# 18281818221/kalle-audio

Hardware: AMD Instinct MI355X
Metric: audio-seconds/sec (node) DiT train step, 10s@12.5Hz x1024 latents (higher is better)
Workload: dtype bf16; 1 GPU; DiT train step (fwd+bwd+allreduce+Adam), 24 blocks D=1536 h=24, 10 s @ 12.5 Hz x 1024 latents (T=125+1 prepend), S=130 x 768 cross-attn cond; DiT shape chosen by this build (reference defines none); global_batch=256, per_gpu_batch=256, parallelism=dp1, objective=v, io_channels=1024, global_cond_type=prepend

## Files before the change

kalle_audio_amd/csrc/gemm2.hip:

```cpp
#include <stdio.h>
#include <stdlib.h>
#include <string.h>

#include <algorithm>
#include <functional>
#include <type_traits>
#include <utility>

#include "gemm_common.h"
#include "../../include/kalle_hip.h"

namespace {

constexpr int BK2 = 64;
#define GPTR(p) ((const __attribute__((address_space(1))) void*)(p))

__device__ __attribute__((aligned(64))) const unsigned kalle_zero_block[16] = {0, 0, 0, 0, 0, 0, 0, 0, 0, 0, 0, 0, 0, 0, 0, 0};

template <bool KM, int R, int NW>
struct Loader {
    static constexpr int PER_WAVE = (R / 8) / NW;
    const bf16_t* src[PER_WAVE];
    int64_t kstep;

// ... 51 lines not shown
            __builtin_amdgcn_global_load_lds(GPTR(sp), LDS_PTR(void, region + (wave * PER_WAVE + i) * 1024), 16, 0, 0);
            src[i] += kstep;
        }
    }
    __device__ __forceinline__ void issue_at(char* region, int wave, int lane, int t, int tail_t, int kvalid) {
        if (t == tail_t) issue_tail(region, wave, lane, kvalid);
        else issue(region, wave);
    }
};

template <int OFF>
__device__ __forceinline__ i32x4 lds_b128(unsigned a) {
    i32x4 r;
    asm volatile("ds_read_b128 %0, %1 offset:%2" : "=v"(r) : "v"(a), "n"(OFF));
    return r;
}
__device__ __forceinline__ i32x2 lds_tr(unsigned a) {
    i32x2 r;
    asm volatile("ds_read_b64_tr_b16 %0, %1" : "=v"(r) : "v"(a));
    return r;
}

template <bool KM, int R>
struct Reader {
    unsigned b0[2], b1[2];
    __device__ __forceinline__ void init(int region_off, int rbase, int lane) {
#pragma unroll
        for (int s = 0; s < 2; ++s) {
            if constexpr (!KM) {
                const int row = rbase + (lane & 15);
                const int c = 4 * s + (lane >> 4);
                b0[s] = region_off + row * 128 + ((c ^ ((row >> 1) & 7)) << 4);
                b1[s] = 0;
            } else {
                constexpr int RB = 2 * R;
                const int g = lane >> 4, i = lane & 15;
                const int q = i >> 2, pp = i & 3;
                const int b = 4 * s + g;
                const int odd = b & 1;
                const int pos1 = 8 * b + (odd ? 4 : 0) + q;
                const int pos2 = 8 * b + (odd ? 0 : 4) + q;
                const int cl = (rbase >> 3) + (pp >> 1);
                const int hb = (pp & 1) * 8;
                b0[s] = region_off + pos1 * RB + ((cl ^ (2 * (pos1 & 7))) << 4) + hb;
                b1[s] = region_off + pos2 * RB + ((cl ^ (2 * (pos2 & 7))) << 4) + hb;
            }
        }
    }
    template <int S, int NTILE, int T0 = 0>
    __device__ __forceinline__ void read(unsigned so, i32x4 (&f)[NTILE]) const {
        if constexpr (!KM) {
            const unsigned a = b0[S] + so;
            f[0] = lds_b128<2048 * (T0 + 0)>(a);
            f[1] = lds_b128<2048 * (T0 + 1)>(a);
            f[2] = lds_b128<2048 * (T0 + 2)>(a);
            f[3] = lds_b128<2048 * (T0 + 3)>(a);
            if constexpr (NTILE == 8) {
                f[4] = lds_b128<2048 * (T0 + 4)>(a);
                f[5] = lds_b128<2048 * (T0 + 5)>(a);
                f[6] = lds_b128<2048 * (T0 + 6)>(a);
                f[7] = lds_b128<2048 * (T0 + 7)>(a);
            }
        } else {
            const unsigned a0 = b0[S] + so, a1 = b1[S] + so;
#pragma unroll
            for (int t = 0; t < NTILE; ++t) {
                const i32x2 lo = lds_tr(a0 ^ ((T0 + t) << 5));
                const i32x2 hi = lds_tr(a1 ^ ((T0 + t) << 5));
                f[t] = i32x4{lo[0], lo[1], hi[0], hi[1]};
            }
        }
    }
};

__device__ __forceinline__ void gemm_stamp(const GemmParams& p, int wave, int lane, int idx, int slot = -1) {
    if (p.stamps && (wave == 0 || wave == 7) && lane == 0)
        p.stamps[((int64_t)(slot < 0 ? (int)blockIdx.x : slot) * 2 + (wave ? 1 : 0)) * 8 + idx] = __builtin_amdgcn_s_memrealtime();
}

constexpr int EPI_DEPTH = 1;

struct NoHook { __device__ __forceinline__ void operator()() const {} };

__device__ __forceinline__ int pidx(int r, int c) { return r * 64 + (c ^ ((r & 1) << 2)); }

template <bool C_F32, int TM, int GLU = 0, typename Hook = NoHook>
__device__ __forceinline__ void wave_epilogue(const GemmParams& p, f32x4 (&acc)[TM][4], char* patch_base, int wave, int lane,
                                              int row0, int col0, Hook after_barrier = Hook{}, int stamp_slot = -1) {
    constexpr int DEPTH = EPI_DEPTH < TM ? EPI_DEPTH : TM;
    float* patch = reinterpret_cast<float*>(patch_base) + wave * (16 * 64);
    const int g = lane >> 4, li = lane & 15;
    const bool pre_res = C_F32 && GLU == 0 && !p.atomic && p.residual != nullptr;
    f32x4 rbuf[DEPTH][4];
    auto load_res = [&](int mt, f32x4 (&rv)[4]) {
#pragma unroll
        for (int i = 0; i < 4; ++i) {
            const int gm = row0 + 16 * mt + g + 4 * i, gn = col0 + 4 * li;
            rv[i] = f32x4{0.f, 0.f, 0.f, 0.f};
            if (gm < p.M && gn < p.N) rv[i] = *reinterpret_cast<const f32x4*>(p.residual + gemm_crow(p, gm) * p.ldr + gn);
        }
    };
    i32x4 hbuf[DEPTH][2][2];
    auto load_h = [&](int mt, i32x4 (&hv)[2][2]) {
        const int c8 = (lane & 7) * 8, j0 = col0 + c8;
#pragma unroll
        for (int half = 0; half < 2; ++half) {
            const int gm = row0 + 16 * mt + (lane >> 3) + 8 * half;
            hv[half][0] = i32x4{0, 0, 0, 0};
            hv[half][1] = i32x4{0, 0, 0, 0};
            if (gm < p.M && j0 < p.glu_inner) {
                const bf16_t* hp = static_cast<const bf16_t*>(p.glu_aux) + (int64_t)gm * 2 * p.glu_inner;
                hv[half][0] = *reinterpret_cast<const i32x4*>(hp + j0);
                hv[half][1] = *reinterpret_cast<const i32x4*>(hp + p.glu_inner + j0);
            }
        }
    };
    asm volatile("s_waitcnt lgkmcnt(0)" ::: "memory");
    __builtin_amdgcn_s_barrier();
    after_barrier();
    gemm_stamp(p, wave, lane, 3, stamp_slot);
#pragma unroll
    for (int d = 0; d < DEPTH; ++d) {
        if constexpr (GLU == 2) load_h(d, hbuf[d]);
        if (pre_res) load_res(d, rbuf[d]);
    }
    float sx[8], sg[8];
#pragma unroll
    for (int e = 0; e < 8; ++e) { sx[e] = 0.f; sg[e] = 0.f; }
    f32x4 bias4 = f32x4{0.f, 0.f, 0.f, 0.f}, bias8[2] = {f32x4{0.f, 0.f, 0.f, 0.f}, f32x4{0.f, 0.f, 0.f, 0.f}};
    float bx[8], bg[8];
#pragma unroll
    for (int e = 0; e < 8; ++e) { bx[e] = 0.f; bg[e] = 0.f; }
    if (p.bias) {
        if constexpr (GLU == 1) {
            const int j0 = col0 + (lane & 3) * 8;
            if (j0 < p.glu_inner) {
#pragma unroll
                for (int e = 0; e < 8; ++e) { bx[e] = p.bias[j0 + e]; bg[e] = p.bias[p.glu_inner + j0 + e]; }
            }
        } else if constexpr (GLU == 0) {
            if constexpr (C_F32) {
                if (!p.atomic && col0 + 4 * li < p.N) bias4 = *reinterpret_cast<const f32x4*>(p.bias + col0 + 4 * li);
            } else {
                const int gn = col0 + 8 * (lane & 7);
                if (gn < p.N) {
                    bias8[0] = *reinterpret_cast<const f32x4*>(p.bias + gn);
                    bias8[1] = *reinterpret_cast<const f32x4*>(p.bias + gn + 4);
                }
            }
        }
    }
#pragma unroll
    for (int mt = 0; mt < TM; ++mt) {
        const int slot = mt % DEPTH;
        f32x4 rcur[4];
        i32x4 hcur[2][2];
        if constexpr (GLU == 2) {
#pragma unroll
            for (int half = 0; half < 2; ++half) { hcur[half][0] = hbuf[slot][half][0]; hcur[half][1] = hbuf[slot][half][1]; }
            if (mt + DEPTH < TM) load_h(mt + DEPTH, hbuf[slot]);
        }
        if (pre_res) {
#pragma unroll
            for (int i = 0; i < 4; ++i) rcur[i] = rbuf[slot][i];
            if (mt + DEPTH < TM) load_res(mt + DEPTH, rbuf[slot]);
        }
#pragma unroll
        for (int nt = 0; nt < 4; ++nt)
#pragma unroll
            for (int r = 0; r < 4; ++r) patch[pidx(4 * g + r, 16 * nt + li)] = acc[mt][nt][r];
        asm volatile("s_waitcnt lgkmcnt(0)" ::: "memory");
        const int rbase = row0 + 16 * mt;
        if constexpr (GLU == 1) {
            const int r = lane >> 2, c8 = (lane & 3) * 8;
            const int gm = rbase + r, j0 = col0 + c8;
            if (gm < p.M && j0 < p.glu_inner) {
                float xv[8], gv[8];
#pragma unroll
                for (int e = 0; e < 8; ++e) { xv[e] = patch[pidx(r, c8 + e)]; gv[e] = patch[pidx(r, 32 + c8 + e)]; }
#pragma unroll
                for (int e = 0; e < 8; ++e) { xv[e] += bx[e]; gv[e] += bg[e]; }
                i32x4 hx, hg, av;
#pragma unroll
                for (int e = 0; e < 4; ++e) {
                    hx[e] = (int)pack_bf16x2(xv[2 * e], xv[2 * e + 1]);
                    hg[e] = (int)pack_bf16x2(gv[2 * e], gv[2 * e + 1]);
                    const float x0 = bf16lo((uint32_t)hx[e]), x1 = bf16hi((uint32_t)hx[e]);
                    const float g0 = bf16lo((uint32_t)hg[e]), g1 = bf16hi((uint32_t)hg[e]);
                    av[e] = (int)pack_bf16x2(x0 * siluf_(g0), x1 * siluf_(g1));
                }
                bf16_t* hp = reinterpret_cast<bf16_t*>(p.C) + (int64_t)gm * p.ldc;
                *reinterpret_cast<i32x4*>(hp + j0) = hx;
                *reinterpret_cast<i32x4*>(hp + p.glu_inner + j0) = hg;
                *reinterpret_cast<i32x4*>(static_cast<bf16_t*>(p.glu_aux) + (int64_t)gm * p.glu_inner + j0) = av;
            }
        } else if constexpr (GLU == 2) {
            const int c8 = (lane & 7) * 8, j0 = col0 + c8;
#pragma unroll
            for (int half = 0; half < 2; ++half) {
                const int r = (lane >> 3) + 8 * half;
                const int gm = rbase + r;
                if (gm < p.M && j0 < p.glu_inner) {
                    const i32x4 xv = hcur[half][0], gv = hcur[half][1];
                    i32x4 ox, og;
#pragma unroll
                    for (int e = 0; e < 4; ++e) {
                        const float x[2] = {bf16lo((uint32_t)xv[e]), bf16hi((uint32_t)xv[e])};
                        const float gg[2] = {bf16lo((uint32_t)gv[e]), bf16hi((uint32_t)gv[e])};
                        const float d[2] = {bf16_to_f32(f32_to_bf16(patch[pidx(r, c8 + 2 * e)] * p.alpha)),
                                            bf16_to_f32(f32_to_bf16(patch[pidx(r, c8 + 2 * e + 1)] * p.alpha))};
                        float dx[2], dg[2];
#pragma unroll
                        for (int q = 0; q < 2; ++q) {
                            const float sgm = sigmoidf_(gg[q]);
                            dx[q] = d[q] * gg[q] * sgm;
                            dg[q] = d[q] * x[q] * sgm * (1.f + gg[q] * (1.f - sgm));
                        }
                        ox[e] = (int)pack_bf16x2(dx[0], dx[1]);
                        og[e] = (int)pack_bf16x2(dg[0], dg[1]);
                        sx[2 * e] += bf16lo((uint32_t)ox[e]); sx[2 * e + 1] += bf16hi((uint32_t)ox[e]);
                        sg[2 * e] += bf16lo((uint32_t)og[e]); sg[2 * e + 1] += bf16hi((uint32_t)og[e]);
                    }
                    bf16_t* dp = reinterpret_cast<bf16_t*>(p.C) + (int64_t)gm * p.ldc;
                    *reinterpret_cast<i32x4*>(dp + j0) = ox;
                    *reinterpret_cast<i32x4*>(dp + p.glu_inner + j0) = og;
                }
            }
        } else if (p.atomic) {
            const int gn = col0 + lane;
#pragma unroll 4
            for (int r = 0; r < 16; ++r) {
                const int gm = rbase + r;
                if (gm < p.M && gn < p.N)
                    atomicAdd(reinterpret_cast<float*>(p.C) + (int64_t)gm * p.ldc + gn, patch[pidx(r, lane)] * p.alpha);
            }
        } else if constexpr (C_F32) {
#pragma unroll
            for (int i = 0; i < 4; ++i) {
                const int r = g + 4 * i;
                const int gm = rbase + r, gn = col0 + 4 * li;
                if (gm >= p.M || gn >= p.N) continue;
                const f32x4 pv = *reinterpret_cast<const f32x4*>(patch + pidx(r, 4 * li));
                float v[4] = {pv[0], pv[1], pv[2], pv[3]};
                const int64_t crow = gemm_crow(p, gm);
                gemm_epilogue4(p, gm, gn, crow, v, false, &bias4);
                if (pre_res) {
#pragma unroll
                    for (int j = 0; j < 4; ++j) v[j] += rcur[i][j];
                }
                float* cp = reinterpret_cast<float*>(p.C) + crow * p.ldc + gn;
                if (p.accumulate) {
                    const f32x4 c0 = *reinterpret_cast<const f32x4*>(cp);
#pragma unroll
                    for (int j = 0; j < 4; ++j) v[j] += c0[j];
                }
                *reinterpret_cast<f32x4*>(cp) = f32x4{v[0], v[1], v[2], v[3]};
            }
        } else {
#pragma unroll
            for (int half = 0; half < 2; ++half) {
                const int r = (lane >> 3) + 8 * half;
                const int gm = rbase + r, gn = col0 + 8 * (lane & 7);
                if (gm >= p.M || gn >= p.N) continue;
                const f32x4 p0 = *reinterpret_cast<const f32x4*>(patch + pidx(r, 8 * (lane & 7)));
                const f32x4 p1 = *reinterpret_cast<const f32x4*>(patch + pidx(r, 8 * (lane & 7) + 4));
                float v0[4] = {p0[0], p0[1], p0[2], p0[3]}, v1[4] = {p1[0], p1[1], p1[2], p1[3]};
                const int64_t crow = gemm_crow(p, gm);
                gemm_epilogue4(p, gm, gn, crow, v0, true, &bias8[0]);
                gemm_epilogue4(p, gm, gn + 4, crow, v1, true, &bias8[1]);
                i32x4 o;
                o[0] = (int)pack_bf16x2(v0[0], v0[1]);
                o[1] = (int)pack_bf16x2(v0[2], v0[3]);
                o[2] = (int)pack_bf16x2(v1[0], v1[1]);
                o[3] = (int)pack_bf16x2(v1[2], v1[3]);
                *reinterpret_cast<i32x4*>(reinterpret_cast<bf16_t*>(p.C) + crow * p.ldc + gn) = o;
            }
        }
        asm volatile("s_waitcnt lgkmcnt(0)" ::: "memory");
    }
    if constexpr (GLU == 2) {
        if (p.glu_dbias) {
#pragma unroll
            for (int e = 0; e < 8; ++e) {
#pragma unroll
                for (int o = 8; o < 64; o <<= 1) { sx[e] += __shfl_xor(sx[e], o, 64); sg[e] += __shfl_xor(sg[e], o, 64); }
            }
            const int j0 = col0 + (lane & 7) * 8;
            if (lane < 8 && j0 < p.glu_inner) {
#pragma unroll
                for (int e = 0; e < 8; ++e) {
                    atomicAdd(p.glu_dbias + j0 + e, sx[e]);
                    atomicAdd(p.glu_dbias + p.glu_inner + j0 + e, sg[e]);
                }
            }
        }
    }
    if (p.stamps) {
        gemm_stamp(p, wave, lane, 4, stamp_slot);
        asm volatile("s_waitcnt vmcnt(0)" ::: "memory");
        gemm_stamp(p, wave, lane, 5, stamp_slot);
    }
}

#define MFMA16(FA, FB)                                                                                         \
    _Pragma("unroll") for (int mt = 0; mt < 4; ++mt) _Pragma("unroll") for (int nt = 0; nt < 4; ++nt)          \
        acc[mt][nt] = __builtin_amdgcn_mfma_f32_16x16x32_bf16(__builtin_bit_cast(bf16x8, FA[mt]),              \
                                                              __builtin_bit_cast(bf16x8, FB[nt]), acc[mt][nt], 0, 0, 0)

template <bool A_KM, bool B_KM, bool C_F32, int WM, int WN, int TM, int GLU = 0, int NS = 3>
__global__ __launch_bounds__(WM * WN * 64, 2) void gemm2_kernel(GemmParams p) {
    static_assert(TM == 4, "wave tile is 64 x 64");
    constexpr int TN = 4;
    constexpr int NW = WM * WN;
    constexpr int BM = WM * TM * 16, BN = WN * TN * 16;
    constexpr int A_BYTES = BM * 128, B_BYTES = BN * 128, STAGE = A_BYTES + B_BYTES;
    extern __shared__ __attribute__((aligned(16))) char smem[];
    const unsigned lds0 = (unsigned)(size_t)LDS_PTR(char, smem);

    const int tid = threadIdx.x, lane = tid & 63;
    const int wave = __builtin_amdgcn_readfirstlane(tid >> 6);
    const int wm = wave / WN, wn = wave % WN;

    int tm, tn;
    gemm_tile_coords(blockIdx.x, gridDim.x, p.tiles_m, p.tiles_n, p.group_m, tm, tn);
    const int m0 = tm * BM, n0 = tn * BN;

    const int nk_all = (p.K + BK2 - 1) / BK2;
    const int kt0 = blockIdx.y * p.ktiles_per_split;
    const int nk = min(p.ktiles_per_split, nk_all - kt0);
    const int kvalid = p.K % BK2;
    const int tail_t = kvalid ? nk_all - 1 - kt0 : -1;

    f32x4 acc[TM][TN];
#pragma unroll
    for (int i = 0; i < TM; ++i)
#pragma unroll
        for (int j = 0; j < TN; ++j) acc[i][j] = f32x4{0.f, 0.f, 0.f, 0.f};

    Loader<A_KM, BM, NW> la;
    Loader<B_KM, BN, NW> lb;
    la.init(p.A, p.lda, p.M, m0, kt0 * BK2, wave, lane);
    lb.init(p.B, p.ldb, p.N, n0, kt0 * BK2, wave, lane, GLU == 1 ? p.glu_inner : 0, tn);
    const int arow = wm * TM * 16, bcol = wn * TN * 16;
    Reader<A_KM, BM> ra;
    Reader<B_KM, BN> rb;
    ra.init(lds0, arow, lane);
    rb.init(lds0 + A_BYTES, bcol, lane);

    {
    constexpr int PT = Loader<A_KM, BM, NW>::PER_WAVE + Loader<B_KM, BN, NW>::PER_WAVE;
    static_assert((NS - 2) * PT <= 63, "vmcnt is a 6-bit counter");
    {
        const int pre = nk < NS ? nk : NS;
#pragma unroll
        for (int t = 0; t < NS; ++t) {
            if (t < pre) {
                la.issue_at(smem + t * STAGE, wave, lane, t, tail_t, kvalid);
                lb.issue_at(smem + t * STAGE + A_BYTES, wave, lane, t, tail_t, kvalid);
            }
        }
        constexpr int PRE_KEEP = (NS - 1) * PT <= 63 ? NS - 1 : NS - 2;
        const int keep = pre - 1 < PRE_KEEP ? pre - 1 : PRE_KEEP;
        auto wait_keep = [&](auto self, auto c) {
            constexpr int C = decltype(c)::value;
            if (keep == C) asm volatile("s_waitcnt vmcnt(%0)" ::"n"(C * PT) : "memory");
            if constexpr (C > 0) self(self, std::integral_constant<int, C - 1>{});
        };
        wait_keep(wait_keep, std::integral_constant<int, PRE_KEEP>{});
    }
    __builtin_amdgcn_s_barrier();
    __builtin_amdgcn_sched_barrier(0);

    i32x4 fa0[4], fb0[4], fa1[4], fb1[4];
    ra.template read<0, 4>(0, fa0);
    rb.template read<0, 4>(0, fb0);

    unsigned so_cur = 0, so_nxt = STAGE;
    int kt = 0;

    auto iteration = [&](auto issue_c, auto next_c, auto keep_c) {
        constexpr bool ISSUE = decltype(issue_c)::value, NEXT = decltype(next_c)::value;
        constexpr int KEEP = decltype(keep_c)::value;
        asm volatile("s_waitcnt lgkmcnt(0)" ::: "memory");
        __builtin_amdgcn_sched_barrier(0);
        ra.template read<1, 4>(so_cur, fa1);
        rb.template read<1, 4>(so_cur, fb1);
        __builtin_amdgcn_sched_barrier(0);
        MFMA16(fa0, fb0);
        __builtin_amdgcn_sched_barrier(0);
        asm volatile("s_waitcnt vmcnt(%0) lgkmcnt(0)" ::"n"(KEEP * PT) : "memory");
        __builtin_amdgcn_s_barrier();
        __builtin_amdgcn_sched_barrier(0);
        if (wave >= NW / 2) {
            MFMA16(fa1, fb1);
            __builtin_amdgcn_sched_barrier(0);
        }
        if constexpr (ISSUE) {
            la.issue_at(smem + so_cur, wave, lane, kt + NS, tail_t, kvalid);
            lb.issue_at(smem + so_cur + A_BYTES, wave, lane, kt + NS, tail_t, kvalid);
        }
        if constexpr (NEXT) {
            ra.template read<0, 4>(so_nxt, fa0);
            rb.template read<0, 4>(so_nxt, fb0);
        }
        __builtin_amdgcn_sched_barrier(0);
        if (wave < NW / 2) {
            MFMA16(fa1, fb1);
            __builtin_amdgcn_sched_barrier(0);
        }
        so_cur = so_nxt;
        so_nxt = so_nxt + STAGE >= NS * STAGE ? 0 : so_nxt + STAGE;
    };
    using T_ = std::true_type;
    using F_ = std::false_type;
#pragma unroll 1
    for (; kt + NS < nk; ++kt) iteration(T_{}, T_{}, std::integral_constant<int, NS - 2>{});
    auto tail = [&](auto self, auto r) {
        constexpr int R = decltype(r)::value;
        if (nk - 1 - kt == R) { iteration(F_{}, T_{}, std::integral_constant<int, R - 1>{}); ++kt; }
        if constexpr (R > 1) self(self, std::integral_constant<int, R - 1>{});
    };
    tail(tail, std::integral_constant<int, NS - 1>{});
    iteration(F_{}, F_{}, std::integral_constant<int, 0>{});
    }

    if constexpr (C_F32) {
        if (p.slab_stride) {
            GemmParams q = p;
            q.C = static_cast<float*>(p.C) + (int64_t)blockIdx.y * p.slab_stride;
            wave_epilogue<C_F32, TM>(q, acc, smem, wave, lane, m0 + arow, n0 + bcol);
            return;
        }
    }
    wave_epilogue<C_F32, TM, GLU>(p, acc, smem, wave, lane, m0 + arow, GLU == 1 ? tn * (BN / 2) + wn * 32 : n0 + bcol);
}


template <bool B_KM, bool C_F32, int WM, int WN, int GLU, int NS>
__global__ __launch_bounds__(WM * WN * 128, 1) void gemm2_ks2_kernel(GemmParams p) {
    static_assert(!B_KM || WN >= 2, "a k-major operand tile needs >= 128 columns (16 swizzle slots per k-row)");
    constexpr int TM = 4, TN = 4;
    constexpr int NWT = WM * WN, NW = 2 * NWT;
    constexpr int BM = WM * 64, BN = WN * 64;
    constexpr int A_BYTES = BM * 128, B_BYTES = BN * 128, STAGE = A_BYTES + B_BYTES;
    constexpr int RED_OFF = 32768;
    static_assert(RED_OFF + NWT * 16384 <= NS * STAGE, "partial-sum exchange must fit into the ring");
    extern __shared__ __attribute__((aligned(16))) char smem[];
    const unsigned lds0 = (unsigned)(size_t)LDS_PTR(char, smem);

    const int tid = threadIdx.x, lane = tid & 63;
    const int wave = __builtin_amdgcn_readfirstlane(tid >> 6);
    const int kg = wave / NWT, wt = wave % NWT;
    const int wm = wt / WN, wn = wt % WN;

    int tm, tn;
    gemm_tile_coords(blockIdx.x, gridDim.x, p.tiles_m, p.tiles_n, p.group_m, tm, tn);
    const int m0 = tm * BM, n0 = tn * BN;

    const int nk_all = (p.K + BK2 - 1) / BK2;
    const int kt0 = blockIdx.y * p.ktiles_per_split;
    const int nk = min(p.ktiles_per_split, nk_all - kt0);
    const int kvalid = p.K % BK2;
    const int tail_t = kvalid ? nk_all - 1 - kt0 : -1;

    f32x4 acc[TM][TN];
#pragma unroll
    for (int i = 0; i < TM; ++i)
#pragma unroll
        for (int j = 0; j < TN; ++j) acc[i][j] = f32x4{0.f, 0.f, 0.f, 0.f};

    Loader<false, BM, NW> la;
    Loader<B_KM, BN, NW> lb;
    la.init(p.A, p.lda, p.M, m0, kt0 * BK2, wave, lane);
    lb.init(p.B, p.ldb, p.N, n0, kt0 * BK2, wave, lane, GLU == 1 ? p.glu_inner : 0, tn);
    const int arow = wm * 64, bcol = wn * 64;
    Reader<false, BM> ra;
    Reader<B_KM, BN> rb;
    ra.init(lds0, arow, lane);
    rb.init(lds0 + A_BYTES, bcol, lane);

    constexpr int PT = Loader<false, BM, NW>::PER_WAVE + Loader<B_KM, BN, NW>::PER_WAVE;
    static_assert((NS - 1) * PT <= 63, "vmcnt is a 6-bit counter");
    {
        const int pre = nk < NS ? nk : NS;
#pragma unroll
        for (int t = 0; t < NS; ++t) {
            if (t < pre) {
                la.issue_at(smem + t * STAGE, wave, lane, t, tail_t, kvalid);
                lb.issue_at(smem + t * STAGE + A_BYTES, wave, lane, t, tail_t, kvalid);
            }
        }
        const int keep = pre - 1;
        auto wait_keep = [&](auto self, auto c) {
            constexpr int C = decltype(c)::value;
            if (keep == C) asm volatile("s_waitcnt vmcnt(%0)" ::"n"(C * PT) : "memory");
            if constexpr (C > 0) self(self, std::integral_constant<int, C - 1>{});
        };
        wait_keep(wait_keep, std::integral_constant<int, NS - 1>{});
    }
    __builtin_amdgcn_s_barrier();
    __builtin_amdgcn_sched_barrier(0);

    i32x4 fa[2][4], fb[2][4];
    auto rd = [&](unsigned so, i32x4 (&A)[4], i32x4 (&B)[4]) {
        if (kg == 0) { ra.template read<0, 4>(so, A); rb.template read<0, 4>(so, B); }
        else { ra.template read<1, 4>(so, A); rb.template read<1, 4>(so, B); }
    };
    rd(0, fa[0], fb[0]);
    unsigned so_cur = 0, so_nxt = STAGE;
    int kt = 0;

    auto iteration = [&](auto par_c, auto issue_c, auto next_c, auto keep_c) {
        constexpr int P = decltype(par_c)::value, KEEP = decltype(keep_c)::value;
        constexpr bool ISSUE = decltype(issue_c)::value, NEXT = decltype(next_c)::value;
        asm volatile("s_waitcnt vmcnt(%0) lgkmcnt(0)" ::"n"(KEEP * PT) : "memory");
        __builtin_amdgcn_s_barrier();
        __builtin_amdgcn_sched_barrier(0);
        if constexpr (NEXT) rd(so_nxt, fa[1 - P], fb[1 - P]);
        __builtin_amdgcn_sched_barrier(0);
        MFMA16(fa[P], fb[P]);
        __builtin_amdgcn_sched_barrier(0);
        if constexpr (ISSUE) {
            la.issue_at(smem + so_cur, wave, lane, kt + NS, tail_t, kvalid);
            lb.issue_at(smem + so_cur + A_BYTES, wave, lane, kt + NS, tail_t, kvalid);
        }
        so_cur = so_nxt;
        so_nxt = so_nxt + STAGE >= NS * STAGE ? 0 : so_nxt + STAGE;
    };
    using T_ = std::true_type;
    using F_ = std::false_type;
    using P0 = std::integral_constant<int, 0>;
    using P1 = std::integral_constant<int, 1>;
    using KS_ = std::integral_constant<int, NS - 2>;
#pragma unroll 1
    for (; kt + NS + 1 < nk; kt += 2) {
        iteration(P0{}, T_{}, T_{}, KS_{});
        ++kt; iteration(P1{}, T_{}, T_{}, KS_{}); --kt;
    }
    int par = 0;
    if (kt + NS < nk) { iteration(P0{}, T_{}, T_{}, KS_{}); ++kt; par = 1; }
    auto tail = [&](auto self, auto r) {
        constexpr int R = decltype(r)::value;
        if (nk - 1 - kt == R) {
            if (par) iteration(P1{}, F_{}, T_{}, std::integral_constant<int, R - 1>{});
            else iteration(P0{}, F_{}, T_{}, std::integral_constant<int, R - 1>{});
            ++kt; par ^= 1;
        }
        if constexpr (R > 1) self(self, std::integral_constant<int, R - 1>{});
    };
    tail(tail, std::integral_constant<int, NS - 1>{});
    if (par) iteration(P1{}, F_{}, F_{}, P0{});
    else iteration(P0{}, F_{}, F_{}, P0{});

    asm volatile("s_waitcnt vmcnt(0) lgkmcnt(0)" ::: "memory");
    __builtin_amdgcn_s_barrier();
    float* red = reinterpret_cast<float*>(smem + RED_OFF) + wt * 4096;
    if (kg == 1) {
#pragma unroll
        for (int i = 0; i < TM; ++i)
#pragma unroll
            for (int j = 0; j < TN; ++j) *reinterpret_cast<f32x4*>(red + ((i * TN + j) * 64 + lane) * 4) = acc[i][j];
    }
    asm volatile("s_waitcnt lgkmcnt(0)" ::: "memory");
    __builtin_amdgcn_s_barrier();
    if (kg == 1) {
        __builtin_amdgcn_s_barrier();
        return;
    }
#pragma unroll
    for (int i = 0; i < TM; ++i)
#pragma unroll
        for (int j = 0; j < TN; ++j) acc[i][j] += *reinterpret_cast<const f32x4*>(red + ((i * TN + j) * 64 + lane) * 4);
    if constexpr (C_F32) {
        if (p.slab_stride) {
            GemmParams q = p;
            q.C = static_cast<float*>(p.C) + (int64_t)blockIdx.y * p.slab_stride;
            wave_epilogue<C_F32, TM>(q, acc, smem, wt, lane, m0 + arow, n0 + bcol);
            return;
        }
    }
    wave_epilogue<C_F32, TM, GLU>(p, acc, smem, wt, lane, m0 + arow, GLU == 1 ? tn * (BN / 2) + wn * 32 : n0 + bcol);
}

template <bool B_KM, bool C_F32, int WM, int WN, int GLU, int NS>
int launch2_ks2(const GemmParams& p, hipStream_t st) {
    constexpr int lds = NS * (WM + WN) * 64 * 128;
    static_assert(lds <= 160 * 1024, "LDS per workgroup");
    static std::atomic<uint64_t> lds_ok{0};
    kalle_allow_lds(reinterpret_cast<const void*>(gemm2_ks2_kernel<B_KM, C_F32, WM, WN, GLU, NS>), lds, lds_ok);
    dim3 grid(p.tiles_m * p.tiles_n, p.splits), block(WM * WN * 128);
    KALLE_LAUNCH((gemm2_ks2_kernel<B_KM, C_F32, WM, WN, GLU, NS>), grid, block, lds, st, p);
    return kalle_check_launch();
}

template <bool A_KM, bool B_KM, bool C_F32, int WM, int WN, int TM, int GLU = 0, int NS = 3>
int launch2(const GemmParams& p, hipStream_t st) {
    constexpr int BM = WM * TM * 16, BN = WN * 64;
    constexpr int lds = NS * (BM + BN) * 128;
    static_assert(lds <= 160 * 1024, "LDS per workgroup");
    static std::atomic<uint64_t> lds_ok{0};
    kalle_allow_lds(reinterpret_cast<const void*>(gemm2_kernel<A_KM, B_KM, C_F32, WM, WN, TM, GLU, NS>), lds, lds_ok);
    dim3 grid(p.tiles_m * p.tiles_n, p.splits), block(WM * WN * 64);
    KALLE_LAUNCH((gemm2_kernel<A_KM, B_KM, C_F32, WM, WN, TM, GLU, NS>), grid, block, lds, st, p);
    return kalle_check_launch();
}



constexpr int GEMM3_LDS = 2 * (256 + 256) * 128 + 8 * 16 * 64 * 4;

static int kalle_cu_count() {
    static std::atomic<int> cached[64];
    int dev = 0;
    (void)hipGetDevice(&dev);
    int v = cached[dev & 63].load(std::memory_order_relaxed);
    if (v > 0) return v;
    hipDeviceProp_t prop;
    v = hipGetDeviceProperties(&prop, dev) == hipSuccess && prop.multiProcessorCount > 0 ? prop.multiProcessorCount : 256;
    v &= ~7;
    if (v < 8) v = 8;
    cached[dev & 63].store(v, std::memory_order_relaxed);
    return v;
}

#define MFMA32(FA, FB)                                                                                         \
    _Pragma("unroll") for (int mt = 0; mt < 8; ++mt) _Pragma("unroll") for (int nt = 0; nt < 4; ++nt)          \
        acc[mt][nt] = __builtin_amdgcn_mfma_f32_16x16x32_bf16(__builtin_bit_cast(bf16x8, FA[mt]),              \
                                                              __builtin_bit_cast(bf16x8, FB[nt]), acc[mt][nt], 0, 0, 0)

constexpr int SCHED_SETS = 256;
constexpr int SCHED_LINE = 32;
__device__ int kalle_gemm_sched[SCHED_SETS][9 * SCHED_LINE];

__device__ __forceinline__ int sched_issue(int* sched, int xcd) { return atomicAdd(sched + xcd * SCHED_LINE, 1); }
__device__ __forceinline__ int sched_resolve(int xcd, int raw, int first_round, int ntiles) {
    const int id = xcd + 8 * (first_round + raw);
    return id < ntiles ? id : ntiles;
}
__device__ __forceinline__ void sched_leave(int* sched, int nwg) {
    if (atomicAdd(sched + 8 * SCHED_LINE, 1) == nwg - 1) {
#pragma unroll
        for (int i = 0; i < 9; ++i) atomicExch(sched + i * SCHED_LINE, 0);
    }
}

template <bool A_KM, bool B_KM, bool C_F32, int GLU, bool XCD_RASTER, bool PERSIST>
__device__ __forceinline__ void gemm3_tiles(const GemmParams& p, int tile0, int tstride, int tile_end, int ntiles_raster, int kt0,
                                            int nk) {
    const int kvalid = p.K % BK2;
    const int tail_t = kvalid ? (p.K + BK2 - 1) / BK2 - 1 - kt0 : -1;
    constexpr int WN = 4, TM = 8, NW = 8;
    constexpr int BM = 256, BN = 256;
    constexpr int A_BYTES = BM * 128, B_BYTES = BN * 128, STAGE = A_BYTES + B_BYTES;
    extern __shared__ __attribute__((aligned(16))) char smem[];
    const unsigned lds0 = (unsigned)(size_t)LDS_PTR(char, smem);

    const int tid = threadIdx.x, lane = tid & 63;
    const int wave = __builtin_amdgcn_readfirstlane(tid >> 6);
    const int wm = wave / WN, wn = wave % WN;
    const int arow = wm * 128, bcol = wn * 64;
    Loader<A_KM, BM, NW> la;
    Loader<B_KM, BN, NW> lb;
    Reader<A_KM, BM> ra;
    Reader<B_KM, BN> rb;
    ra.init(lds0, arow, lane);
    rb.init(lds0 + A_BYTES, bcol, lane);
    const bool late = wave >= NW / 2;
    if (late) __builtin_amdgcn_s_setprio(1);

    auto coords = [&](int tile, int& tm, int& tn) {
        if constexpr (XCD_RASTER) gemm_tile_coords(tile, ntiles_raster, p.tiles_m, p.tiles_n, p.group_m, tm, tn);
        else gemm_tile_coords_plain(tile, p.tiles_m, p.tiles_n, p.group_m, tm, tn);
    };
    auto init_loaders = [&](int tm, int tn, int kt_first) {
        la.init(p.A, p.lda, p.M, tm * BM, (kt0 + kt_first) * BK2, wave, lane);
        lb.init(p.B, p.ldb, p.N, tn * BN, (kt0 + kt_first) * BK2, wave, lane, GLU == 1 ? p.glu_inner : 0, tn);
    };
    bool prefetched = false;
    unsigned s0 = 0;

    int* const sched = PERSIST && p.sched_set > 0 ? &kalle_gemm_sched[p.sched_set - 1][0] : nullptr;
    int next_tile = tile_end;
    int drawn = 0;
    if constexpr (PERSIST) {
        if (sched && tid == 0) drawn = sched_issue(sched, blockIdx.x & 7);
    }
    volatile int* const mailbox = reinterpret_cast<volatile int*>(smem + 2 * STAGE);
    for (int tile = tile0; tile < tile_end; tile = next_tile) {
        int tm, tn;
        coords(tile, tm, tn);
        const int m0 = tm * BM, n0 = tn * BN;
        next_tile = PERSIST ? tile + tstride : tile_end;
        bool has_next = PERSIST && next_tile < tile_end;
        gemm_stamp(p, wave, lane, 0, tile);
        f32x4 acc[TM][4];
#pragma unroll
        for (int i = 0; i < TM; ++i)
#pragma unroll
            for (int j = 0; j < 4; ++j) acc[i][j] = f32x4{0.f, 0.f, 0.f, 0.f};

        if (!prefetched) {
            init_loaders(tm, tn, 0);
            la.issue_at(smem, wave, lane, 0, tail_t, kvalid);
            lb.issue_at(smem + A_BYTES, wave, lane, 0, tail_t, kvalid);
            s0 = 0;
            if (nk > 1) {
                la.issue_at(smem + STAGE, wave, lane, 1, tail_t, kvalid);
                lb.issue_at(smem + STAGE + A_BYTES, wave, lane, 1, tail_t, kvalid);
                asm volatile("s_waitcnt vmcnt(8)" ::: "memory");
            } else {
                asm volatile("s_waitcnt vmcnt(0)" ::: "memory");
            }
        } else if constexpr (PERSIST) {
            init_loaders(tm, tn, nk > 1 ? 2 : 1);
            asm volatile("s_waitcnt vmcnt(0)" ::: "memory");
        }
        if constexpr (PERSIST) {
            if (sched && tid == 0) {
                *mailbox = sched_resolve(blockIdx.x & 7, drawn, tstride >> 3, tile_end);
                asm volatile("s_waitcnt lgkmcnt(0)" ::: "memory");
            }
        }
        __builtin_amdgcn_s_barrier();
        __builtin_amdgcn_sched_barrier(0);
        if constexpr (PERSIST) {
            if (sched) {
                next_tile = __builtin_amdgcn_readfirstlane(*mailbox);
                has_next = next_tile < tile_end;
            }
        }
        gemm_stamp(p, wave, lane, 1, tile);

        i32x4 fa[8], fb[4];
        unsigned so_cur = s0;
        int kt = 0;
        ra.template read<0, 8>(so_cur, fa);
        rb.template read<0, 4>(so_cur, fb);

        auto iteration = [&](auto issue_c, auto next_c) {
            constexpr bool ISSUE = decltype(issue_c)::value, NEXT = decltype(next_c)::value;
            asm volatile("s_waitcnt lgkmcnt(0)" ::: "memory");
            __builtin_amdgcn_sched_barrier(0);
            MFMA32(fa, fb);
            __builtin_amdgcn_sched_barrier(0);
            ra.template read<1, 8>(so_cur, fa);
            rb.template read<1, 4>(so_cur, fb);
            asm volatile("s_waitcnt lgkmcnt(0)" ::: "memory");
            __builtin_amdgcn_sched_barrier(0);
            if (!late) {
                MFMA32(fa, fb);
                __builtin_amdgcn_sched_barrier(0);
            }
            asm volatile("s_waitcnt vmcnt(0)" ::: "memory");
            __builtin_amdgcn_s_barrier();
            __builtin_amdgcn_sched_barrier(0);
            if (late) {
                MFMA32(fa, fb);
                __builtin_amdgcn_sched_barrier(0);
            }
            if constexpr (ISSUE) {
                la.issue_at(smem + so_cur, wave, lane, kt + 2, tail_t, kvalid);
                lb.issue_at(smem + so_cur + A_BYTES, wave, lane, kt + 2, tail_t, kvalid);
            }
            so_cur ^= STAGE;
            if constexpr (NEXT) {
                ra.template read<0, 8>(so_cur, fa);
                rb.template read<0, 4>(so_cur, fb);
            }
            __builtin_amdgcn_sched_barrier(0);
        };
        auto last_iteration = [&]() {
            asm volatile("s_waitcnt lgkmcnt(0)" ::: "memory");
            __builtin_amdgcn_sched_barrier(0);
            MFMA32(fa, fb);
            __builtin_amdgcn_sched_barrier(0);
            ra.template read<1, 8>(so_cur, fa);
            rb.template read<1, 4>(so_cur, fb);
            asm volatile("s_waitcnt lgkmcnt(0)" ::: "memory");
            __builtin_amdgcn_sched_barrier(0);
            MFMA32(fa, fb);
            __builtin_amdgcn_sched_barrier(0);
        };
        using T_ = std::true_type;
        using F_ = std::false_type;
#pragma unroll 1
        for (; kt + 2 < nk; ++kt) iteration(T_{}, T_{});
        if (kt + 1 < nk) { iteration(F_{}, T_{}); ++kt; }
        if constexpr (!PERSIST || GLU == 2) iteration(F_{}, F_{});
        else last_iteration();
        gemm_stamp(p, wave, lane, 2, tile);

        const unsigned s_last = so_cur;
        auto hook = [&]() {
            if constexpr (!PERSIST) return;
            if (has_next) {
                int ntm, ntn;
                coords(next_tile, ntm, ntn);
                init_loaders(ntm, ntn, 0);
                la.issue_at(smem + (s_last ^ STAGE), wave, lane, 0, tail_t, kvalid);
                lb.issue_at(smem + (s_last ^ STAGE) + A_BYTES, wave, lane, 0, tail_t, kvalid);
                if (nk > 1) {
                    la.issue_at(smem + s_last, wave, lane, 1, tail_t, kvalid);
                    lb.issue_at(smem + s_last + A_BYTES, wave, lane, 1, tail_t, kvalid);
                }
                if (sched && tid == 0) drawn = sched_issue(sched, blockIdx.x & 7);
            }
        };
        wave_epilogue<C_F32, TM, GLU>(p, acc, smem + 2 * STAGE, wave, lane, m0 + arow, GLU == 1 ? tn * 128 + wn * 32 : n0 + bcol,
                                      hook, tile);
        prefetched = has_next;
        s0 = s_last ^ STAGE;
        if constexpr (!PERSIST) break;
    }
}

template <bool A_KM, bool B_KM, bool C_F32, int GLU = 0>
__global__ __launch_bounds__(512, 2) void gemm3_kernel(GemmParams p) {
    const int nk_all = (p.K + BK2 - 1) / BK2;
    const int ntiles = p.tiles_m * p.tiles_n;
    if constexpr (A_KM) {
        if (p.mix_na >= 0) {
            const int na = p.mix_na, sa = p.mix_sa;
            int bid = blockIdx.x, tile, slice, per;
            if (bid < na * sa) { tile = bid % na; slice = bid / na; per = (nk_all + sa - 1) / sa; }
            else { bid -= na * sa; const int nb = ntiles - na; tile = na + bid % nb; slice = bid / nb; per = (nk_all + sa) / (sa + 1); }
            const int kt0 = slice * per, nk = min(per, nk_all - kt0);
            if (nk <= 0) return;
            gemm3_tiles<A_KM, B_KM, C_F32, GLU, true, false>(p, tile, 0, tile + 1, ntiles, kt0, nk);
        } else {
            const int kt0 = blockIdx.y * p.ktiles_per_split;
            gemm3_tiles<A_KM, B_KM, C_F32, GLU, true, false>(p, blockIdx.x, 0, blockIdx.x + 1, ntiles, kt0,
                                                             min(p.ktiles_per_split, nk_all - kt0));
        }
    } else {
        gemm3_tiles<A_KM, B_KM, C_F32, GLU, true, true>(p, blockIdx.x, gridDim.x, ntiles, ntiles, 0, nk_all);
        if (p.sched_set > 0 && threadIdx.x == 0) sched_leave(&kalle_gemm_sched[p.sched_set - 1][0], gridDim.x);
    }
}

struct GroupProblem {
    const bf16_t* A;
    const bf16_t* B;
    float* C;
    int64_t lda, ldb, ldc;
    int M, N, K;
    int tiles_m, tiles_n, group_m;
    int unsplit, splits;
    int r1_start, r2_start;
};
struct GroupParams {
    int nprob, r2_base;
    int overwrite;
    GroupProblem pr[KALLE_MAX_GROUP];
};

__global__ __launch_bounds__(256) void gemm3_group_zero_kernel(GroupParams gp) {
    int pi = 0, base = 0;
    const int bid = blockIdx.x >> 2, band = blockIdx.x & 3;
    for (;;) {
        const int nb = gp.pr[pi].tiles_m * gp.pr[pi].tiles_n - gp.pr[pi].unsplit;
        if (bid < base + nb || pi + 1 >= gp.nprob) break;
        base += nb;
        ++pi;
    }
    const GroupProblem& q = gp.pr[pi];
    int tm, tn;
    gemm_tile_coords_plain(q.unsplit + bid - base, q.tiles_m, q.tiles_n, q.group_m, tm, tn);
    const int r0 = tm * 256 + band * 64, c0 = tn * 256;
    for (int i = threadIdx.x; i < 64 * 64; i += 256) {
        const int r = r0 + i / 64, c = c0 + (i & 63) * 4;
        if (r < q.M && c < q.N) *reinterpret_cast<f32x4*>(q.C + (int64_t)r * q.ldc + c) = f32x4{0.f, 0.f, 0.f, 0.f};
    }
}

__global__ __launch_bounds__(512, 2) void gemm3_wgrad_group_kernel(GroupParams gp) {
    const bool whole = (int)blockIdx.x < gp.r2_base;
    const int bid = whole ? xcd_contiguous(blockIdx.x, gp.r2_base)
                          : gp.r2_base + xcd_contiguous(blockIdx.x - gp.r2_base, gridDim.x - gp.r2_base);
    int pi = 0, tile, slice = 0;
    if (whole) {
        while (pi + 1 < gp.nprob && bid >= gp.pr[pi + 1].r1_start) ++pi;
        tile = bid - gp.pr[pi].r1_start;
    } else {
        while (pi + 1 < gp.nprob && bid >= gp.pr[pi + 1].r2_start) ++pi;
        const int local = bid - gp.pr[pi].r2_start, nb = gp.pr[pi].tiles_m * gp.pr[pi].tiles_n - gp.pr[pi].unsplit;
        tile = gp.pr[pi].unsplit + local % nb;
        slice = local / nb;
    }
    const GroupProblem& q = gp.pr[pi];
    GemmParams p{};
    p.A = q.A; p.B = q.B; p.C = q.C;
    p.lda = q.lda; p.ldb = q.ldb; p.ldc = q.ldc;
    p.M = q.M; p.N = q.N; p.K = q.K;
    p.alpha = 1.f;
    p.rows_per_batch = 1;
    p.accumulate = gp.overwrite ? 0 : 1;
    p.atomic = whole ? 0 : 1;
    const int ntiles = q.tiles_m * q.tiles_n, nk_all = (q.K + BK2 - 1) / BK2;
    p.tiles_m = q.tiles_m; p.tiles_n = q.tiles_n; p.group_m = q.group_m;
    int kt0 = 0, nk = nk_all;
    if (!whole) {
        const int per = (nk_all + q.splits - 1) / q.splits;
        kt0 = slice * per;
        nk = min(per, nk_all - kt0);
        if (nk <= 0) return;
    }
    gemm3_tiles<true, true, true, 0, false, false>(p, tile, 0, tile + 1, ntiles, kt0, nk);
}

template <bool A_KM, bool B_KM, bool C_F32, int GLU = 0>
int launch3(const GemmParams& p, hipStream_t st) {
    constexpr int lds = GEMM3_LDS;
    static std::atomic<uint64_t> lds_ok{0};
    kalle_allow_lds(reinterpret_cast<const void*>(gemm3_kernel<A_KM, B_KM, C_F32, GLU>), lds, lds_ok);
    dim3 grid(p.tiles_m * p.tiles_n, p.splits), block(512);
    if (p.mix_na >= 0) {
        const int ntiles = p.tiles_m * p.tiles_n;
        grid = dim3(p.mix_na * p.mix_sa + (ntiles - p.mix_na) * (p.mix_sa + 1), 1);
    } else if (!A_KM) {
        if (p.splits != 1) return KALLE_ERR_UNSUPPORTED;
        const int cus = kalle_cu_count();
        if ((int)grid.x > cus) {
            GemmParams q = p;
            grid.x = cus;
            static std::atomic<unsigned> next_set{0};
            hipStreamCaptureStatus cap = hipStreamCaptureStatusNone;
            const bool capturing = hipStreamIsCapturing(st, &cap) == hipSuccess && cap != hipStreamCaptureStatusNone;
            q.sched_set = !capturing ? 1 + (int)(next_set.fetch_add(1, std::memory_order_relaxed) % SCHED_SETS) : 0;
            KALLE_LAUNCH((gemm3_kernel<A_KM, B_KM, C_F32, GLU>), grid, block, lds, st, q);
            return kalle_check_launch();
        }
    }
    KALLE_LAUNCH((gemm3_kernel<A_KM, B_KM, C_F32, GLU>), grid, block, lds, st, p);
    return kalle_check_launch();
}

int launch3_layout(const GemmParams& p, bool a_km, bool b_km, bool f32, hipStream_t st) {
    if (!a_km && !b_km) return f32 ? launch3<false, false, true>(p, st) : launch3<false, false, false>(p, st);
    if (!a_km && b_km) return f32 ? launch3<false, true, true>(p, st) : launch3<false, true, false>(p, st);
    if (a_km && b_km) return launch3<true, true, true>(p, st);
    return KALLE_ERR_UNSUPPORTED;
}

template <int WM, int WN, int TM>
int launch2_layout(const GemmParams& p, bool a_km, bool b_km, bool f32, hipStream_t st) {
    if (!a_km && !b_km) return f32 ? launch2<false, false, true, WM, WN, TM>(p, st) : launch2<false, false, false, WM, WN, TM>(p, st);
    if (!a_km && b_km) return f32 ? launch2<false, true, true, WM, WN, TM>(p, st) : launch2<false, true, false, WM, WN, TM>(p, st);
    if (a_km && b_km) return launch2<true, true, true, WM, WN, TM>(p, st);
    return KALLE_ERR_UNSUPPORTED;
}

struct CuReplay {
    double cu[256] = {};
    void run(int tiles, int nk, int slices) {
        if (tiles <= 0 || slices <= 0) return;
        const int per = (nk + slices - 1) / slices;
        for (int sl = 0; sl < slices; ++sl) {
            const int k = nk - sl * per < per ? nk - sl * per : per;
            if (k <= 0) break;
            const double d = 10.0 + 1.6 * k;
            for (int t = 0; t < tiles; ++t) {
                std::pop_heap(cu, cu + 256, std::greater<double>());
                cu[255] += d;
                std::push_heap(cu, cu + 256, std::greater<double>());
            }
        }
    }
    double makespan() const {
        double mk = 0.0;
        for (int c = 0; c < 256; ++c) mk = cu[c] > mk ? cu[c] : mk;
        return mk;
    }
};

inline bool al16(const void* p) { return (reinterpret_cast<uintptr_t>(p) & 15) == 0; }

}

int kalle_gemm_v2_launch(GemmParams& p, bool a_km, bool b_km, bool f32, hipStream_t st) {
    p.mix_na = -1;
    p.mix_sa = 0;
    if (p.K & 7) return KALLE_ERR_UNSUPPORTED;
    if (a_km && !b_km) return KALLE_ERR_UNSUPPORTED;
    if (a_km && !f32) return KALLE_ERR_UNSUPPORTED;
    if (p.M < 256 || p.N < 128) return KALLE_ERR_UNSUPPORTED;
    if (a_km && (p.M & 7)) return KALLE_ERR_UNSUPPORTED;
    const int nk = (p.K + BK2 - 1) / BK2;
    if (p.glu_mode) {
        if (a_km || f32 || p.gate || p.residual || p.row_mask || p.c_rpb || p.accumulate) return KALLE_ERR_UNSUPPORTED;
        if (p.glu_inner % 128 || p.N != (p.glu_mode == 1 ? 2 * p.glu_inner : p.glu_inner)) return KALLE_ERR_UNSUPPORTED;
        if (p.glu_mode == 1 && b_km) return KALLE_ERR_UNSUPPORTED;
        if (p.glu_mode == 2 && (!b_km || p.bias)) return KALLE_ERR_UNSUPPORTED;
        p.tiles_m = (p.M + 255) / 256;
        p.tiles_n = p.glu_mode == 1 ? p.glu_inner / 128 : (p.glu_inner + 255) / 256;
        p.tile_n = 256;
        p.group_m = p.tiles_m < 4 ? p.tiles_m : 4;
        p.splits = 1;
        p.atomic = 0;
        p.ktiles_per_split = nk;
        if (p.glu_mode == 1) return launch3<false, false, false, 1>(p, st);
        return launch3<false, true, false, 2>(p, st);
    }
    const bool plain = !p.bias && !p.gate && !p.residual && !p.row_mask && p.c_rpb == 0;
    const bool can_split = f32 && plain && a_km && nk >= 16;
    const double flops = 2.0 * p.M * p.N * p.K;
    double best = 1e30;
    int best_bn = 128, best_s = 1;
    for (int bn = 128; bn <= 256; bn += 128) {
        if (bn == 256 && p.N < 256) continue;
        const double rate = bn == 256 ? 1150e12 : 1000e12;
        const int tiles = ((p.M + 255) / 256) * ((p.N + bn - 1) / bn);
        for (int s = 1; s <= (can_split ? 16 : 1) && (s == 1 || nk / s >= 8); ++s) {
            const int blocks = tiles * s;
            const double eff = (double)blocks / (((blocks + 255) / 256) * 256.0);
            const double t = flops / (rate * eff) + (s > 1 ? (double)s * p.M * p.N * 4.0 / 2.0e12 : 0.0);
            if (t < best * 0.98) { best = t; best_bn = bn; best_s = s; }
        }
    }
    if (can_split && best_bn == 256) {
        struct Plan { int M, N, kb, sa, na; };
        static thread_local Plan cache[32];
        static thread_local int ncache = 0, victim = 0;
        const Plan* hit = nullptr;
        int sa_sel = 0, na_sel = -1;
        for (int i = 0; i < ncache; ++i)
            if (cache[i].M == p.M && cache[i].N == p.N && cache[i].kb == nk / 16) hit = &cache[i];
        if (!hit) {
            const int ntiles = ((p.M + 255) / 256) * ((p.N + 255) / 256);
            auto replay = [&](int sa, int na) {
                CuReplay r;
                r.run(na, nk, sa);
                r.run(ntiles - na, nk, sa + 1);
                const double savg = ((double)na * sa + (double)(ntiles - na) * (sa + 1)) / ntiles;
                return r.makespan() + (savg > 1.0 ? savg * p.M * p.N * 4.0 / 2.0e12 * 1e6 : 0.0);
            };
            Plan best_plan{p.M, p.N, nk / 16, 0, -1};
            double t_uniform = 1e30, t_best = 1e30;
            const int step = ntiles / 12 > 4 ? (ntiles / 12 + 3) & ~3 : 4;
            for (int sl = 1; sl <= 16 && (sl == 1 || nk / sl >= 8); ++sl) {
                const double t = replay(sl - 1, 0);
                if (t < t_uniform) t_uniform = t;
            }
            for (int sa = best_s > 3 ? best_s - 3 : 1; sa <= best_s + 1 && sa <= 15; ++sa) {
                if (nk / (sa + 1) < 8) break;
                for (int na = step; na < ntiles; na += step) {
                    const double t = replay(sa, na);
                    if (t < t_best) { t_best = t; best_plan.sa = sa; best_plan.na = na; }
                }
            }
            if (!(best_plan.na > 0 && t_best < 0.97 * t_uniform)) best_plan.na = -1;
            if (ncache < 32) cache[ncache++] = best_plan;
            else { cache[victim] = best_plan; victim = (victim + 1) & 31; }
            sa_sel = best_plan.sa;
            na_sel = best_plan.na;
        } else {
            sa_sel = hit->sa;
            na_sel = hit->na;
        }
        if (na_sel > 0 && nk / (sa_sel + 1) < 8) na_sel = -1;
        if (na_sel > 0) { p.mix_na = na_sel; p.mix_sa = sa_sel; best_s = sa_sel + 1; }
    }
    p.tiles_m = (p.M + 255) / 256;
    p.tiles_n = (p.N + best_bn - 1) / best_bn;
    p.tile_n = best_bn;
    p.group_m = p.tiles_m < 4 ? p.tiles_m : 4;
    p.splits = best_s;
    p.atomic = best_s > 1;
    if (p.atomic && !p.accumulate) {
        if (hipMemset2DAsync(p.C, p.ldc * sizeof(float), 0, p.N * sizeof(float), p.M, st) != hipSuccess)
            return KALLE_ERR_LAUNCH;
    }
    p.ktiles_per_split = (nk + p.splits - 1) / p.splits;
    p.splits = (nk + p.ktiles_per_split - 1) / p.ktiles_per_split;
    if (best_bn == 256) return launch3_layout(p, a_km, b_km, f32, st);
    return launch2_layout<4, 2, 4>(p, a_km, b_km, f32, st);
}

namespace {
template <bool C_F32>
__global__ __launch_bounds__(256) void gemm_finish_kernel(GemmParams p, const float* __restrict__ ws, int nslab) {
    const int64_t slab = (int64_t)p.M * p.N;
    auto ld4 = [&](int64_t off) {
        f32x4 a = *reinterpret_cast<const f32x4*>(ws + off);
        for (int s = 1; s < nslab; ++s) {
            const f32x4 b = *reinterpret_cast<const f32x4*>(ws + s * slab + off);
            a[0] += b[0]; a[1] += b[1]; a[2] += b[2]; a[3] += b[3];
        }
        return a;
    };
    const int cols4 = (p.glu_mode == 1 ? p.glu_inner : p.N) >> 2;
    const int64_t total = (int64_t)p.M * cols4;
    for (int64_t i = (int64_t)blockIdx.x * blockDim.x + threadIdx.x; i < total; i += (int64_t)gridDim.x * blockDim.x) {
        const int gm = (int)(i / cols4), gn = (int)(i - (int64_t)gm * cols4) * 4;
        if (p.glu_mode == 1) {
            const f32x4 xv = ld4((int64_t)gm * p.N + gn);
            const f32x4 gv = ld4((int64_t)gm * p.N + p.glu_inner + gn);
            float x[4] = {xv[0], xv[1], xv[2], xv[3]}, g[4] = {gv[0], gv[1], gv[2], gv[3]};
            if (p.bias) {
#pragma unroll
                for (int j = 0; j < 4; ++j) { x[j] += p.bias[gn + j]; g[j] += p.bias[p.glu_inner + gn + j]; }
            }
            i32x2 hx, hg, av;
#pragma unroll
            for (int e = 0; e < 2; ++e) {
                hx[e] = (int)pack_bf16x2(x[2 * e], x[2 * e + 1]);
                hg[e] = (int)pack_bf16x2(g[2 * e], g[2 * e + 1]);
                const float x0 = bf16lo((uint32_t)hx[e]), x1 = bf16hi((uint32_t)hx[e]);
                const float g0 = bf16lo((uint32_t)hg[e]), g1 = bf16hi((uint32_t)hg[e]);
                av[e] = (int)pack_bf16x2(x0 * siluf_(g0), x1 * siluf_(g1));
            }
            bf16_t* hp = reinterpret_cast<bf16_t*>(p.C) + (int64_t)gm * p.ldc;
            *reinterpret_cast<i32x2*>(hp + gn) = hx;
// ... 327 lines not shown
```

Before: 11740 audio-seconds/sec.

## Write bf16 GEMM epilogue directly from registers via transposed MFMA and permlane swap

For persistent non-GLU bf16-output GEMMs with row-major A, the MFMA operands are swapped so each lane holds a contiguous run of columns. A permlane16 swap then assembles 8 bf16 values per lane, which are stored straight to global memory. This skips staging the accumulators through LDS in the epilogue, saving LDS traffic and LDS space and letting the next tile's prefetch overlap better. The trade-off is extra lane permutes and a lane-to-column mapping that must match the bias and epilogue indexing to stay correct.

```diff
diff --git a/kalle_audio_amd/csrc/gemm2.hip b/kalle_audio_amd/csrc/gemm2.hip
--- a/kalle_audio_amd/csrc/gemm2.hip
+++ b/kalle_audio_amd/csrc/gemm2.hip
@@ -377,6 +377,57 @@
     }
 }
 
+
+__device__ __forceinline__ i32x4 pair_swap8(uint32_t a0, uint32_t a1, uint32_t b0, uint32_t b1) {
+    const auto lo = __builtin_amdgcn_permlane16_swap(a0, b0, false, false);
+    const auto hi = __builtin_amdgcn_permlane16_swap(a1, b1, false, false);
+    return i32x4{(int)lo[0], (int)hi[0], (int)lo[1], (int)hi[1]};
+}
+
+template <int TM, typename Hook>
+__device__ __forceinline__ void wave_epilogue_regs(const GemmParams& p, f32x4 (&acc)[TM][4], int wave, int lane, int row0, int col0,
+                                                   Hook after_barrier, int stamp_slot) {
+    const int g = lane >> 4, li = lane & 15;
+    const int cb = 16 * (g & 1) + 4 * (g & ~1);
+    asm volatile("s_waitcnt lgkmcnt(0)" ::: "memory");
+    __builtin_amdgcn_s_barrier();
+    after_barrier();
+    gemm_stamp(p, wave, lane, 3, stamp_slot);
+    f32x4 bias4[4];
+#pragma unroll
+    for (int nt = 0; nt < 4; ++nt) {
+        const int gn = col0 + 16 * nt + 4 * g;
+        bias4[nt] = f32x4{0.f, 0.f, 0.f, 0.f};
+        if (p.bias && gn < p.N) bias4[nt] = *reinterpret_cast<const f32x4*>(p.bias + gn);
+    }
+#pragma unroll
+    for (int mt = 0; mt < TM; ++mt) {
+        const int gm = row0 + 16 * mt + li;
+        const bool row_ok = gm < p.M;
+        const int64_t crow = gemm_crow(p, gm);
+        uint32_t w[4][2];
+#pragma unroll
+        for (int nt = 0; nt < 4; ++nt) {
+            const int gn = col0 + 16 * nt + 4 * g;
+            float v[4] = {acc[mt][nt][0], acc[mt][nt][1], acc[mt][nt][2], acc[mt][nt][3]};
+            if (row_ok && gn < p.N) gemm_epilogue4(p, gm, gn, crow, v, true, &bias4[nt]);
+            w[nt][0] = pack_bf16x2(v[0], v[1]);
+            w[nt][1] = pack_bf16x2(v[2], v[3]);
+        }
+#pragma unroll
+        for (int pr = 0; pr < 2; ++pr) {
+            const i32x4 o = pair_swap8(w[2 * pr][0], w[2 * pr][1], w[2 * pr + 1][0], w[2 * pr + 1][1]);
+            const int gn = col0 + 32 * pr + cb;
+            if (row_ok && gn < p.N) *reinterpret_cast<i32x4*>(reinterpret_cast<bf16_t*>(p.C) + crow * p.ldc + gn) = o;
+        }
+    }
+    if (p.stamps) {
+        gemm_stamp(p, wave, lane, 4, stamp_slot);
+        asm volatile("s_waitcnt vmcnt(0)" ::: "memory");
+        gemm_stamp(p, wave, lane, 5, stamp_slot);
+    }
+}
+
 #define MFMA16(FA, FB)                                                                                         \
     _Pragma("unroll") for (int mt = 0; mt < 4; ++mt) _Pragma("unroll") for (int nt = 0; nt < 4; ++nt)          \
         acc[mt][nt] = __builtin_amdgcn_mfma_f32_16x16x32_bf16(__builtin_bit_cast(bf16x8, FA[mt]),              \
@@ -703,6 +754,18 @@
         acc[mt][nt] = __builtin_amdgcn_mfma_f32_16x16x32_bf16(__builtin_bit_cast(bf16x8, FA[mt]),              \
                                                               __builtin_bit_cast(bf16x8, FB[nt]), acc[mt][nt], 0, 0, 0)
 
+#define MFMA32T(FA, FB)                                                                                        \
+    _Pragma("unroll") for (int mt = 0; mt < 8; ++mt) _Pragma("unroll") for (int nt = 0; nt < 4; ++nt)          \
+        acc[mt][nt] = __builtin_amdgcn_mfma_f32_16x16x32_bf16(__builtin_bit_cast(bf16x8, FB[nt]),              \
+                                                              __builtin_bit_cast(bf16x8, FA[mt]), acc[mt][nt], 0, 0, 0)
+#define MFMA32X(FA, FB)                                                                                        \
+    do {                                                                                                       \
+        if constexpr (REG_EPI) { MFMA32T(FA, FB); } else { MFMA32(FA, FB); }                                   \
+    } while (0)
+
+template <bool C_F32, int GLU>
+constexpr bool gemm3_reg_epilogue() { return !C_F32 && GLU == 0; }
+
 constexpr int SCHED_SETS = 256;
 constexpr int SCHED_LINE = 32;
 __device__ int kalle_gemm_sched[SCHED_SETS][9 * SCHED_LINE];
@@ -726,6 +789,7 @@
     const int tail_t = kvalid ? (p.K + BK2 - 1) / BK2 - 1 - kt0 : -1;
     constexpr int WN = 4, TM = 8, NW = 8;
     constexpr int BM = 256, BN = 256;
+    constexpr bool REG_EPI = PERSIST && !A_KM && gemm3_reg_epilogue<C_F32, GLU>();
     constexpr int A_BYTES = BM * 128, B_BYTES = BN * 128, STAGE = A_BYTES + B_BYTES;
     extern __shared__ __attribute__((aligned(16))) char smem[];
     const unsigned lds0 = (unsigned)(size_t)LDS_PTR(char, smem);
@@ -816,21 +880,21 @@
             constexpr bool ISSUE = decltype(issue_c)::value, NEXT = decltype(next_c)::value;
             asm volatile("s_waitcnt lgkmcnt(0)" ::: "memory");
             __builtin_amdgcn_sched_barrier(0);
-            MFMA32(fa, fb);
+            MFMA32X(fa, fb);
             __builtin_amdgcn_sched_barrier(0);
             ra.template read<1, 8>(so_cur, fa);
             rb.template read<1, 4>(so_cur, fb);
             asm volatile("s_waitcnt lgkmcnt(0)" ::: "memory");
             __builtin_amdgcn_sched_barrier(0);
             if (!late) {
-                MFMA32(fa, fb);
+                MFMA32X(fa, fb);
                 __builtin_amdgcn_sched_barrier(0);
             }
             asm volatile("s_waitcnt vmcnt(0)" ::: "memory");
             __builtin_amdgcn_s_barrier();
             __builtin_amdgcn_sched_barrier(0);
             if (late) {
-                MFMA32(fa, fb);
+                MFMA32X(fa, fb);
                 __builtin_amdgcn_sched_barrier(0);
             }
             if constexpr (ISSUE) {
@@ -847,13 +911,13 @@
         auto last_iteration = [&]() {
             asm volatile("s_waitcnt lgkmcnt(0)" ::: "memory");
             __builtin_amdgcn_sched_barrier(0);
-            MFMA32(fa, fb);
+            MFMA32X(fa, fb);
             __builtin_amdgcn_sched_barrier(0);
             ra.template read<1, 8>(so_cur, fa);
             rb.template read<1, 4>(so_cur, fb);
             asm volatile("s_waitcnt lgkmcnt(0)" ::: "memory");
             __builtin_amdgcn_sched_barrier(0);
-            MFMA32(fa, fb);
+            MFMA32X(fa, fb);
             __builtin_amdgcn_sched_barrier(0);
         };
         using T_ = std::true_type;
@@ -881,8 +945,11 @@
                 if (sched && tid == 0) drawn = sched_issue(sched, blockIdx.x & 7);
             }
         };
-        wave_epilogue<C_F32, TM, GLU>(p, acc, smem + 2 * STAGE, wave, lane, m0 + arow, GLU == 1 ? tn * 128 + wn * 32 : n0 + bcol,
-                                      hook, tile);
+        if constexpr (REG_EPI)
+            wave_epilogue_regs<TM>(p, acc, wave, lane, m0 + arow, n0 + bcol, hook, tile);
+        else
+            wave_epilogue<C_F32, TM, GLU>(p, acc, smem + 2 * STAGE, wave, lane, m0 + arow, GLU == 1 ? tn * 128 + wn * 32 : n0 + bcol,
+                                          hook, tile);
         prefetched = has_next;
         s0 = s_last ^ STAGE;
         if constexpr (!PERSIST) break;
```

Measured after the change: 11790 audio-seconds/sec (median of 6 runs). No clear change (+0.4%).
